# tiantianxuabc/ORB_SLAM2_Refactored

Measured on AMD Instinct MI355X. Metric: frames/sec ORB extract+match (1280×720, 8 lvl, 1000 feat) + LocalBA iters/sec, higher is better.
Workload: dtype u8; 1 GPU; C2: 1280x720 mono, 8 levels, 2000 features, extract + brute-force Hamming top-2/ratio match of every frame vs its predecessor; width=1280, height=720, nlevels=8, nfeatures=2000, parallelism=8192-frame job sharded over 1 GPU(s), 8192 frames per GPU

## Files before the change

### orb_slam2_refactored_amd/csrc/orbx.hip

```cpp
#include <algorithm>
#include <cfloat>
#include <cmath>
#include <cstring>
#include <mutex>
#include <type_traits>
#include <vector>

#include <hip/hip_ext.h>

#include "common.h"
#include "qt_sort.h"
#include "sincos_f.h"
#include "stereo.h"

#include "orbx_geom.h"
#include "orbx_pyramid.h"
#include "orbx_fast.h"
#include "orbx_quadtree.h"
#include "orbx_describe.h"

using namespace orbamd;

struct orbx_extractor {
    orbx_params p;
    int device = 0;
    hipStream_t stream = nullptr;
    std::vector<float> scale, inv_scale, sigma2, inv_sigma2;
    std::vector<int> quota;
    std::mutex mu;

    int g_rows = -1, g_cols = -1;
    Geom geom;
    std::vector<CellDev> cells;
    int NC = 0, PTC = 0;
    size_t qt_lds = 0;
    int qt_ptc0 = 0;
    size_t qt_lds0 = 0;
    int qt_wave = 0, qt_wave_wg = 2, qtw_l0 = 0, qtw_nc = 0, qtw_ptc = 0;
    size_t qtw_lds = 0;
    FastLds fl;
    size_t fast_lds = 0;
    int fast_cpw = 16;
    int fast_spec = 8;
    int fast_pair = 0;
    bool fast_pair_on = false;
    int fast_spec_first = 1;
    int nsub = 1;
    int debug_nc = 0;
    int debug_qt_block = 0;
    uint32_t fault_host = 0;
    int pyr_mfma = 0;
    std::vector<char> pyr_mfma_ok;
    DevBuf d_pyrmt, d_pyrkb;
    int pyr_pair = 2;
    int trig_float = 0;
    int resize_simd = 0;
    std::vector<std::pair<hipStream_t, hipEvent_t>> sub;
    hipEvent_t fork_ev = nullptr;
    bool lvl_overlap = false;
    hipStream_t lvl_side = nullptr;
    hipEvent_t lvl_fork = nullptr, lvl_join = nullptr;
    DevBuf d_cells, d_xtab, d_ytab;
    DevBuf d_strips;
    DevBuf d_slottab;
    DevBuf d_lvlpre;
    std::vector<int> strip_beg;

    int ws_frames = 0;
    DevBuf d_pyr, d_slots, d_cellcnt, d_P, d_T, d_sel, d_selcnt, d_fault;
    DevBuf d_img, d_kps, d_desc, d_counts;
    DevBuf d_stereo_sad;
    void release_buffers() {
        DevBuf* bufs[] = {&d_cells, &d_strips, &d_xtab, &d_ytab, &d_pyr, &d_slots, &d_cellcnt, &d_P,
                          &d_T, &d_sel, &d_selcnt, &d_fault, &d_img, &d_kps, &d_desc,
                          &d_counts, &d_stereo_sad, &d_pyrmt, &d_pyrkb, &d_slottab, &d_lvlpre,
                          &d_stereo_out, &d_dstat};
        for (DevBuf* b : bufs) b->release();
    }
    int prof = 0;
    std::vector<std::pair<hipEvent_t, hipEvent_t>> prof_ev[4];
    std::vector<hipEvent_t> ev_pool;
    const uint8_t* last_in = nullptr;
    long long last_fstride = 0;
    size_t last_step = 0;
    int last_frames = 0;
// ... 44 lines not shown
        nf *= factor;
    }
    h->quota[L - 1] = std::max(p.nfeatures - sum, 0);
}

static int setup_geometry(orbx_extractor* h, int rows, int cols) {
    if (h->g_rows == rows && h->g_cols == cols) return ORB_OK;
    const int Lc = h->p.nlevels;
    Geom g;
    std::memset(&g, 0, sizeof(g));
    g.nlevels = Lc;
    for (int l = Lc; l < MAX_LEVELS; l++) g.lv[l].out_base = INT_MAX;
    std::vector<int2> xtab, ytab;
    std::vector<PyrMfmaLane> mt;
    std::vector<int> mkb;
    std::vector<CellDev> cells;
    long long pyr_off = 0, slot = 0, cand = 0;
    int out = 0, NC = 64;
    int prev_w = cols, prev_h = rows;
    for (int l = 0; l < Lc; l++) {
        LevelDev& L = g.lv[l];
        if (l == 0) {
            L.w = cols; L.h = rows; L.stride = cols; L.off = -1; L.tail_x = cols; L.mt_off = -1;
        } else {
            L.h = cv_round_f(h->inv_scale[l] * rows);
            L.w = cv_round_f(h->inv_scale[l] * cols);
            if (L.w <= 0 || L.h <= 0) {
                set_error("pyramid level collapses to zero size");
                return ORB_EINVAL;
            }
            L.stride = (int)align_up(L.w, 16);
            L.off = pyr_off;
            pyr_off += (long long)align_up((size_t)L.stride * L.h, 256);
            const int sw = prev_w, sh = prev_h, dw = L.w, dh = L.h;
            const double scale_x = 1. / ((double)dw / sw), scale_y = 1. / ((double)dh / sh);
            L.xtab_off = (int)xtab.size();
            L.ytab_off = (int)ytab.size();
            L.ssx = (double)sw / L.w;
            L.ssy = (double)sh / L.h;
            L.tail_x = resize_tail_x(L.w, h->resize_simd);
            int xmax = dw;
            std::vector<int> sxs(dw), a0s(dw), a1s(dw);
            for (int dx = 0; dx < dw; dx++) {
                float fx = (float)((dx + 0.5) * scale_x - 0.5);
                int sx = (int)std::floor(fx);
                fx -= sx;
                if (sx < 0) { fx = 0; sx = 0; }
                if (sx + 1 >= sw) {
                    xmax = std::min(xmax, dx);
                    if (sx >= sw - 1) { fx = 0; sx = sw - 1; }
                }
                sxs[dx] = sx;
                a0s[dx] = std::min(std::max(cv_round_f((1.f - fx) * 2048), -32768), 32767);
                a1s[dx] = std::min(std::max(cv_round_f(fx * 2048), -32768), 32767);
            }
            for (int dx = 0; dx < dw; dx++) {
                int sx0 = sxs[dx], sx1 = std::min(sxs[dx] + 1, sw - 1), a0 = a0s[dx], a1 = a1s[dx];
                if (dx >= xmax) { sx1 = sx0; a0 = 2048; a1 = 0; }
                xtab.push_back(make_int2(sx0 | (sx1 << 16), (a0 & 0xffff) | (a1 << 16)));
            }
            L.mt_off = h->pyr_mfma ? pyr_mfma_tables(xtab.data() + L.xtab_off, dw, mt, mkb) : -1;
            for (int dy = 0; dy < dh; dy++) {
                float fy = (float)((dy + 0.5) * scale_y - 0.5);
                int sy = (int)std::floor(fy);
                fy -= sy;
                const int b0 = std::min(std::max(cv_round_f((1.f - fy) * 2048), -32768), 32767);
                const int b1 = std::min(std::max(cv_round_f(fy * 2048), -32768), 32767);
                auto clip = [&](int y) { return y < 0 ? 0 : (y >= sh ? sh - 1 : y); };
                ytab.push_back(make_int2(clip(sy) | (clip(sy + 1) << 16), (b0 & 0xffff) | (b1 << 16)));
            }
        }
        if (l > 0) {
            const double sc = (double)prev_w / L.w, scy = (double)prev_h / L.h;
            if (sc * PYR_TW + 12 > PYR_SW || scy * PYR_TH + 6 > PYR_SH) {
                set_error("scaleFactor too large for the pyramid tile (max ~1.9)");
                return ORB_EINVAL;
            }
        }
        if (L.w >= 4096 || L.h >= 4096) {
            set_error("image dimensions must be < 4096");
            return ORB_EINVAL;
        }
        prev_w = L.w; prev_h = L.h;
        L.rx = 16; L.ry = 16; L.rw = L.w - 32; L.rh = L.h - 32;
        L.scale = h->scale[l];
        L.size = h->scale[l] * 31;
        L.quota = h->quota[l];
        L.cell_base = (int)cells.size();
        L.ncells = 0;
        L.cand_base = cand;
        L.cand_cap = 0;
        L.nroots = 0;
        L.out_base = out;
        L.out_cap = 0;
        if (L.rw > 0 && L.rh > 0) {
            const int gridw = L.rw / 30, gridh = L.rh / 30;
            if (gridw > 0 && gridh > 0) {
                const int cellw = (int)std::ceil(1. * L.rw / gridw), cellh = (int)std::ceil(1. * L.rh / gridh);
                const int maxx = L.rx + L.rw, maxy = L.ry + L.rh;
                for (int cy = 0, y0 = L.ry; cy < gridh && y0 + 6 < maxy; cy++, y0 += cellh)
                    for (int cx = 0, x0 = L.rx; cx < gridw && x0 + 6 < maxx; cx++, x0 += cellw) {
                        const int y1 = std::min(y0 + cellh + 6, maxy), x1 = std::min(x0 + cellw + 6, maxx);
                        const int zw = x1 - x0 - 6, zh = y1 - y0 - 6;
// ... 90 lines not shown
            h->qtw_nc = ncw;
            h->qtw_ptc = ptcw;
            h->qtw_lds = 4 * ((size_t)ncw * QT_NODE_BYTES + (size_t)ptcw * 8);
            if (h->qtw_lds > 48 * 1024)
                ORB_HIP_TRY(hipFuncSetAttribute((const void*)quadtree_kernel<true>, hipFuncAttributeMaxDynamicSharedMemorySize,
                                                (int)h->qtw_lds));
        }
    }
    int rc;
    if ((rc = h->d_cells.reserve(std::max<size_t>(1, cells.size()) * sizeof(CellDev)))) return rc;
    if ((rc = h->d_xtab.reserve(std::max<size_t>(1, xtab.size()) * sizeof(int2)))) return rc;
    if ((rc = h->d_ytab.reserve(std::max<size_t>(1, ytab.size()) * sizeof(int2)))) return rc;
    if (!cells.empty())
        ORB_HIP_TRY(hipMemcpy(h->d_cells.ptr, cells.data(), cells.size() * sizeof(CellDev), hipMemcpyHostToDevice));
    if (!xtab.empty())
        ORB_HIP_TRY(hipMemcpy(h->d_xtab.ptr, xtab.data(), xtab.size() * sizeof(int2), hipMemcpyHostToDevice));
    if (!ytab.empty())
        ORB_HIP_TRY(hipMemcpy(h->d_ytab.ptr, ytab.data(), ytab.size() * sizeof(int2), hipMemcpyHostToDevice));
    {
        std::vector<uint32_t> st((size_t)g.out_frame, 0u);
        for (int l = 0; l < Lc; l++)
            for (int i = 0; i < g.lv[l].out_cap; i++) st[(size_t)g.lv[l].out_base + i] = (uint32_t)l | ((uint32_t)i << 8);
        if ((rc = h->d_slottab.reserve(st.size() * sizeof(uint32_t)))) return rc;
        ORB_HIP_TRY(hipMemcpy(h->d_slottab.ptr, st.data(), st.size() * sizeof(uint32_t), hipMemcpyHostToDevice));
    }
    if (!mt.empty() && (rc = h->d_pyrmt.reserve(mt.size() * sizeof(PyrMfmaLane)))) return rc;
    if (!mkb.empty() && (rc = h->d_pyrkb.reserve(mkb.size() * sizeof(int)))) return rc;
    if (!mt.empty())
        ORB_HIP_TRY(hipMemcpy(h->d_pyrmt.ptr, mt.data(), mt.size() * sizeof(PyrMfmaLane), hipMemcpyHostToDevice));
    if (!mkb.empty())
        ORB_HIP_TRY(hipMemcpy(h->d_pyrkb.ptr, mkb.data(), mkb.size() * sizeof(int), hipMemcpyHostToDevice));
    h->pyr_mfma_ok.assign(Lc, 0);
    for (int l = 1; l + 1 < Lc; l++) h->pyr_mfma_ok[l] = h->pyr_mfma && pyr_mfma_pair_fits(g, l, mkb, ytab);
    h->geom = g;
    h->cells = cells;
    {
        std::vector<int2> strips;
        h->strip_beg.assign(g.nlevels + 1, 0);
        const int cpw = std::max(1, std::min(h->fast_cpw, 255));
        for (int l = 0; l < g.nlevels; l++) {
            h->strip_beg[l] = (int)strips.size();
            const LevelDev& L = g.lv[l];
            if (L.ncells <= 0) continue;
            const int x00 = cells[L.cell_base].x0y0 & 0xffff;
            int ncx = 0;
            while (ncx < L.ncells && (cells[L.cell_base + ncx].x0y0 >> 16) == (cells[L.cell_base].x0y0 >> 16)) ncx++;
            const int ncy = L.ncells / ncx;
            if (ncx * ncy != L.ncells || (cells[L.cell_base + ncx - 1].x0y0 & 0xffff) < x00) {
                set_error("FAST cell grid is not a rectangle");
                return ORB_EINTERNAL;
            }
            for (int rb = 0; rb < ncy; rb += cpw)
                for (int cx = 0; cx < ncx; cx++) {
                    const int c0 = L.cell_base + rb * ncx + cx, n = std::min(cpw, ncy - rb);
                    for (int k = 1; k < n; k++)
                        if ((cells[c0 + k * ncx].zwzh & 0xffff) != (cells[c0].zwzh & 0xffff)) {
                            set_error("FAST strip with unequal zone widths");
                            return ORB_EINTERNAL;
                        }
                    strips.push_back(make_int2(c0, n | (ncx << 8)));
                }
        }
        h->strip_beg[g.nlevels] = (int)strips.size();
        if ((rc = h->d_strips.reserve(std::max<size_t>(1, strips.size()) * sizeof(int2)))) return rc;
        if (!strips.empty())
            ORB_HIP_TRY(hipMemcpy(h->d_strips.ptr, strips.data(), strips.size() * sizeof(int2), hipMemcpyHostToDevice));
// ... 133 lines not shown
    const unsigned qt_block = h->debug_qt_block ? (unsigned)h->debug_qt_block : (unsigned)QT_THREADS;
    auto quadtree = [&](int l0, int nl, hipStream_t s) {
        if (nl <= 0) return;
        const int lw = std::max(l0, h->qtw_l0), nw_lv = l0 + nl - lw;
        if (nw_lv > 0) {
            launch_timed(h, 2, quadtree_kernel<true>, dim3((unsigned)F, (unsigned)((nw_lv + 3) / 4)), dim3(qt_block),
                         (uint32_t)h->qtw_lds, s, g, cellcnt, slots, h->d_cells.as<CellDev>(), Pb, Tb, sel, selcnt, h->qtw_nc,
                         h->qtw_ptc, fault, lw, nw_lv);
            nl -= nw_lv;
            if (nl <= 0) return;
        }
        if (h->qt_ptc0 > 0 && l0 == 0) {
            launch_timed(h, 2, quadtree_kernel<false>, dim3((unsigned)F, 1u), dim3(qt_block), (uint32_t)h->qt_lds0, s, g,
                         cellcnt, slots, h->d_cells.as<CellDev>(), Pb, Tb, sel, selcnt, h->NC, h->qt_ptc0, fault, 0, 1);
            l0 = 1;
            if (--nl <= 0) return;
        }
        launch_timed(h, 2, quadtree_kernel<false>, dim3((unsigned)F, (unsigned)nl), dim3(qt_block), (uint32_t)h->qt_lds, s,
                     g, cellcnt, slots, h->d_cells.as<CellDev>(), Pb, Tb, sel, selcnt, h->NC, h->PTC, fault, l0, nl);
    };
    auto pyramid = [&](int l) -> int {
        const int first = h->pyr_pair == 2 ? 1 : 2;
        const bool a16 = l > 1 || (((uintptr_t)d_imgs | (uintptr_t)fstride | (uintptr_t)step) & 15) == 0;
        const bool pair = h->pyr_pair && l >= first && (l - first) % 2 == 0 && l + 1 < g.nlevels && a16;
        auto tiles = [&](int lt) {
            return dim3((unsigned)((g.lv[lt].w + PYR_TW - 1) / PYR_TW), (unsigned)((g.lv[lt].h + PYR_TH - 1) / PYR_TH),
                        (unsigned)F);
        };
        if (pair && h->pyr_mfma && h->pyr_mfma_ok[l]) {
            launch_timed(h, 0, pyramid_pair_mfma_kernel, tiles(l + 1), dim3(256), 0u, st, g, l, d_imgs, fstride, step, pyr,
                         h->d_ytab.as<int2>(), h->d_pyrmt.as<PyrMfmaLane>(), h->d_pyrkb.as<int>());
            return 1;
        }
        if (pair && pyr_pair_fits(g, l)) {
            launch_timed(h, 0, pyramid_pair_kernel, tiles(l + 1), dim3(256), 0u, st, g, l, d_imgs, fstride, step, pyr,
                         h->d_xtab.as<int2>(), h->d_ytab.as<int2>());
            return 1;
        }
        launch_timed(h, 0, pyramid_level_kernel, tiles(l), dim3(256), 0u, st, g, l, d_imgs, fstride, step, pyr,
                     h->d_xtab.as<int2>(), h->d_ytab.as<int2>());
        return 0;
    };
    const int nc0 = g.lv[0].ncells;
    if (side && nc0 > 0 && g.nlevels > 1) {
        (void)hipStreamWaitEvent(side, h->lvl_fork, 0);
        fast(0, 1, side);
        quadtree(0, 1, side);
        (void)hipEventRecord(h->lvl_join, side);
        {
            for (int l = 1; l < g.nlevels; l++) l += pyramid(l);
        }
        fast(1, g.nlevels, st);
        quadtree(1, g.nlevels - 1, st);
        (void)hipStreamWaitEvent(st, h->lvl_join, 0);
    } else {
        {
            for (int l = 1; l < g.nlevels; l++) l += pyramid(l);
        }
        fast(0, g.nlevels, st);
        quadtree(0, g.nlevels, st);
    }
    int* lvlpre = h->d_lvlpre.as<int>() + (long long)f0 * LVP;
    hipLaunchKernelGGL(describe_prefix_kernel, dim3((unsigned)((F + 255) / 256)), dim3(256), 0, st, (const int*)selcnt,
                       g.nlevels, F, lvlpre, d_counts, h->d_dstat.as<int>());
    const int rows_max = std::min(g.out_frame, cap);
    const int C = h->desc_dense ? std::max(1, std::min(h->desc_c > 0 ? h->desc_c : rows_max, rows_max)) : 0;
    DescGrid dg{};
    if (C > 0) {
        dg.C = C;
// ... 599 lines not shown
```

### orb_slam2_refactored_amd/csrc/orbx_pyramid.h

```cpp
#pragma once
#include <cmath>
#include <type_traits>
#include <vector>

#include "orbx_geom.h"

namespace orbamd {

typedef unsigned short us2 __attribute__((ext_vector_type(2)));

__device__ __forceinline__ uint32_t htap24(uint32_t h) { return h & 0xffff0u; }
__device__ __forceinline__ uint32_t mulhi24(uint32_t a, uint32_t b) {
    uint32_t r;
    asm("v_mul_hi_u32_u24 %0, %1, %2" : "=v"(r) : "v"(a), "v"(b));
    return r;
}
__device__ __forceinline__ uint32_t vcoef24(int b) { return ((uint32_t)b & 0xfffu) << 12; }
__device__ __forceinline__ uint32_t vtail(uint32_t h0, uint32_t h1, uint32_t b0_24, uint32_t b1_24) {
    return (__umul24(h0, b0_24 >> 12) + __umul24(h1, b1_24 >> 12) + (1u << 21)) >> 22;
}

__device__ __forceinline__ us2 pyr_tap(uint32_t hi, uint32_t lo, uint32_t sel) {
    const uint32_t r = __builtin_amdgcn_perm(hi, lo, sel);
    return *reinterpret_cast<const us2*>(&r);
}

constexpr int PYR_TW = 64, PYR_TH = 64;
constexpr int PYR_SW = 144, PYR_SH = 128;

__device__ __forceinline__ int4 pyr_row_taps(int2 yv, int sy_lo) {
    return make_int4(((yv.x & 0xffff) - sy_lo) * PYR_SW, ((yv.x >> 16) - sy_lo) * PYR_SW, (int)vcoef24(yv.y),
                     (int)vcoef24(yv.y >> 16));
}

__device__ __forceinline__ void pyr_tile_compute(const Geom& g, const LevelDev& L, int f, uint8_t* pyr,
                                                 const uint8_t* S, const int2* xs_t, const int4* ys_t, int tx0,
                                                 int ty0, int tw, int th, int xa) {
    {
        const int q0 = (threadIdx.x & 15) * 4;
        uint32_t sel0[2], sel1[2];
        int wdb[2];
        us2 a0[2], a1[2];
        bool fits = true;
#pragma unroll
        for (int j = 0; j < 2; j++) {
            const int2 xv0 = xs_t[min(q0 + 2 * j, tw - 1)], xv1 = xs_t[min(q0 + 2 * j + 1, tw - 1)];
            const int s00 = (xv0.x & 0xffff) - xa, s01 = (xv0.x >> 16) - xa;
            const int s10 = (xv1.x & 0xffff) - xa, s11 = (xv1.x >> 16) - xa;
            const int wd = s00 >> 2;
            const int e00 = s00 - 4 * wd, e01 = s01 - 4 * wd, e10 = s10 - 4 * wd, e11 = s11 - 4 * wd;
            fits = fits && max(e01, e11) <= 7 && min(e00, e10) >= 0;
            sel0[j] = (uint32_t)e00 | 0x0c00u | ((uint32_t)e01 << 16) | 0x0c000000u;
            sel1[j] = (uint32_t)e10 | 0x0c00u | ((uint32_t)e11 << 16) | 0x0c000000u;
            wdb[j] = 4 * wd;
            a0[j] = *reinterpret_cast<const us2*>(&xv0.y);
            a1[j] = *reinterpret_cast<const us2*>(&xv1.y);
        }
        if (!__syncthreads_or(!fits)) {
            if (q0 >= tw) return;
            const bool full = q0 + 3 < tw;
            uint8_t* dst = pyr + (long long)f * g.pyr_frame_bytes + L.off + tx0 + q0 +
// ... 37 lines not shown
            return;
        }
    }
    const int q0 = (threadIdx.x & 15) * 4;
    if (q0 >= tw) return;
    uint8_t* dbase = pyr + (long long)f * g.pyr_frame_bytes + L.off + tx0 + q0;
#pragma nounroll
    for (int ty = threadIdx.x >> 4; ty < th; ty += 16) {
        const int4 yv = ys_t[ty];
        const int r0 = yv.x, r1 = yv.y;
        const int b0 = yv.z >> 12, b1 = yv.w >> 12;
        uint32_t packed = 0;
#pragma nounroll
        for (int k = 0; k < 4; k++) {
            const int2 xv = xs_t[min(q0 + k, tw - 1)];
            const int sx0 = (xv.x & 0xffff) - xa, sx1 = (xv.x >> 16) - xa, a0 = xv.y & 0xffff, a1 = xv.y >> 16;
            const int h0 = S[r0 + sx0] * a0 + S[r0 + sx1] * a1;
            const int h1 = S[r1 + sx0] * a0 + S[r1 + sx1] * a1;
            const int s0 = min(h0 >> 4, 32767), s1 = min(h1 >> 4, 32767);
            int v = (((s0 * b0) >> 16) + ((s1 * b1) >> 16) + 2) >> 2;
            if (tx0 + q0 + k >= L.tail_x) v = (h0 * b0 + h1 * b1 + (1 << 21)) >> 22;
            packed |= (uint32_t)(v > 255 ? 255 : v) << (8 * k);
        }
        uint8_t* dst = dbase + (long long)(ty0 + ty) * L.stride;
        if (q0 + 3 < tw) *reinterpret_cast<uint32_t*>(dst) = packed;
        else {
            dst[0] = (uint8_t)packed;
            if (q0 + 1 < tw) dst[1] = (uint8_t)(packed >> 8);
            if (q0 + 2 < tw) dst[2] = (uint8_t)(packed >> 16);
        }
    }
}

constexpr int PYR_PF = 5;

struct PyrTile {
    int f, tx0, ty0, tw, th, sy_lo, xa, nc, items, mul;
    const uint8_t* src;
    int sstep;
};

__device__ __forceinline__ PyrTile pyr_tile_geom(const Geom& g, int l, int t, int ntx, int nty, const uint8_t* in,
                                                 long long in_fstride, int in_step, uint8_t* pyr) {
    const LevelDev& L = g.lv[l];
    const LevelDev& Ls = g.lv[l - 1];
    PyrTile T;
    const int per = ntx * nty;
    T.f = t / per;
    const int r = t - T.f * per;
    T.ty0 = (r / ntx) * PYR_TH;
    T.tx0 = (r - (r / ntx) * ntx) * PYR_TW;
    T.tw = min(PYR_TW, L.w - T.tx0);
    T.th = min(PYR_TH, L.h - T.ty0);
    const int sx_lo = max(0, (int)floor((T.tx0 + 0.5) * L.ssx - 0.5) - 2);
    const int sx_hi = min(Ls.w - 1, (int)floor((T.tx0 + T.tw - 0.5) * L.ssx - 0.5) + 2);
    T.sy_lo = max(0, (int)floor((T.ty0 + 0.5) * L.ssy - 0.5) - 2);
    const int sy_hi = min(Ls.h - 1, (int)floor((T.ty0 + T.th - 0.5) * L.ssy - 0.5) + 2);
    T.xa = sx_lo & ~15;
    T.nc = ((sx_hi - T.xa) >> 4) + 1;
    T.items = (sy_hi - T.sy_lo + 1) * T.nc;
    T.mul = ((1 << 20) + T.nc - 1) / T.nc;
    T.src = level_base(g, l - 1, T.f, in, in_fstride, in_step, pyr, &T.sstep);
    auto u = [](int x) { return __builtin_amdgcn_readfirstlane(x); };
    T.f = u(T.f), T.tx0 = u(T.tx0), T.ty0 = u(T.ty0), T.tw = u(T.tw), T.th = u(T.th), T.sy_lo = u(T.sy_lo);
    T.xa = u(T.xa), T.nc = u(T.nc), T.items = u(T.items), T.mul = u(T.mul), T.sstep = u(T.sstep);
    const unsigned long long sp = (unsigned long long)(uintptr_t)T.src;
    T.src = (const uint8_t*)(uintptr_t)(((unsigned long long)(unsigned)u((int)(sp >> 32)) << 32) |
                                        (unsigned)u((int)(unsigned)sp));
    return T;
}

__device__ __forceinline__ int pyr_piece_row(const PyrTile& T, int i) {
    return (int)(__umulhi(((unsigned)i & 0x7ffu) << 12, (unsigned)T.mul & 0xffffffu) & 0x7ffu);
}
__device__ __forceinline__ int mul12(int a, int b) {
    return (int)(((unsigned)a & 0xfffu) * ((unsigned)b & 0xfffu));
}
__device__ __forceinline__ void pyr_piece_load(const PyrTile& T, int i, uint4& v) {
    if (i < T.items) {
        const int rr = pyr_piece_row(T, i), c = i - mul12(rr, T.nc);
        v = *reinterpret_cast<const uint4*>(T.src + __mul24(T.sy_lo + rr, T.sstep) + T.xa + 16 * c);
    }
}

__device__ __forceinline__ void pyr_fetch(const PyrTile& T, int tid, uint4& v0, uint4& v1, uint4& v2, uint4& v3,
                                          uint4& v4) {
    static_assert(PYR_PF == 5, "five pieces per thread");
    pyr_piece_load(T, tid, v0);
    pyr_piece_load(T, tid + 256, v1);
    pyr_piece_load(T, tid + 512, v2);
    pyr_piece_load(T, tid + 768, v3);
    pyr_piece_load(T, tid + 1024, v4);
}

__device__ __forceinline__ void pyr_stage(const PyrTile& T, int tid, uint8_t* S, const uint4& v, int k) {
    const int i = tid + 256 * k;
    if (i < T.items) {
        const int rr = pyr_piece_row(T, i), c = i - mul12(rr, T.nc);
        *reinterpret_cast<uint4*>(&S[mul12(rr, PYR_SW) + 16 * c]) = v;
    }
}

__global__ __launch_bounds__(256) void pyramid_level_kernel(Geom g, int l, const uint8_t* __restrict__ in,
                                                            long long in_fstride, int in_step, uint8_t* pyr,
                                                            const int2* __restrict__ xtab,
                                                            const int2* __restrict__ ytab) {
    __shared__ __attribute__((aligned(16))) uint8_t S[PYR_SH * PYR_SW + 16];
    __shared__ int2 xs_t[PYR_TW];
    __shared__ int4 ys_t[PYR_TH];
    const LevelDev& L = g.lv[l];
    const LevelDev& Ls = g.lv[l - 1];
    const int gx = gridDim.x, gxy = gridDim.x * gridDim.y;
    const int lb = xcd_swizzle(blockIdx.x + gx * blockIdx.y + gxy * blockIdx.z, gxy * gridDim.z);
    const int f = lb / gxy;
    const int tx0 = (lb % gx) * PYR_TW, ty0 = ((lb % gxy) / gx) * PYR_TH;
    const int tw = min(PYR_TW, L.w - tx0), th = min(PYR_TH, L.h - ty0);
    int sstep;
    const uint8_t* src = level_base(g, l - 1, f, in, in_fstride, in_step, pyr, &sstep);
    const int2* xt = xtab + L.xtab_off;
    const int2* yt = ytab + L.ytab_off;
    const int sw = Ls.w, sh = Ls.h;
    const double scx = L.ssx, scy = L.ssy;
    const int sx_lo = max(0, (int)floor((tx0 + 0.5) * scx - 0.5) - 2);
    const int sx_hi = min(sw - 1, (int)floor((tx0 + tw - 0.5) * scx - 0.5) + 2);
    const int sy_lo = max(0, (int)floor((ty0 + 0.5) * scy - 0.5) - 2);
    if ((int)threadIdx.x < tw) xs_t[threadIdx.x] = xt[tx0 + threadIdx.x];
    if ((int)threadIdx.x >= 64 && (int)threadIdx.x - 64 < th)
        ys_t[threadIdx.x - 64] = pyr_row_taps(yt[ty0 + threadIdx.x - 64], sy_lo);
    const int sy_hi = min(sh - 1, (int)floor((ty0 + th - 0.5) * scy - 0.5) + 2);
    const int xa = sx_lo & ~3;
    const int nd = (sx_hi - xa + 4) >> 2;
    const int nr = sy_hi - sy_lo + 1;
    const bool aligned = ((reinterpret_cast<uintptr_t>(src) | (uintptr_t)sstep) & 3) == 0;
    if (((reinterpret_cast<uintptr_t>(src) | (uintptr_t)sstep) & 15) == 0 && sx_hi - (sx_lo & ~15) < PYR_SW) {
        const PyrTile T = pyr_tile_geom(g, l, lb, gx, gridDim.y, in, in_fstride, in_step, pyr);
        uint4 v0, v1, v2, v3, v4;
        pyr_fetch(T, threadIdx.x, v0, v1, v2, v3, v4);
        pyr_stage(T, threadIdx.x, S, v0, 0);
        pyr_stage(T, threadIdx.x, S, v1, 1);
        pyr_stage(T, threadIdx.x, S, v2, 2);
        pyr_stage(T, threadIdx.x, S, v3, 3);
        pyr_stage(T, threadIdx.x, S, v4, 4);
        __syncthreads();
        pyr_tile_compute(g, L, f, pyr, S, xs_t, ys_t, tx0, ty0, tw, th, T.xa);
        return;
    }
    if (aligned) {
        constexpr int RPW = PYR_SH / 4;
        const int wv = __builtin_amdgcn_readfirstlane((int)(threadIdx.x >> 6));
        const int ln = threadIdx.x & 63;
        const int col = min(xa + 4 * ln, (sw - 1) & ~3);
        const uint8_t* rbase = src + (long long)sy_lo * sstep + col;
        uint32_t v[RPW];
#pragma unroll
        for (int k = 0; k < RPW; k++) {
            const int rk = min(wv + 4 * k, nr - 1);
            v[k] = *reinterpret_cast<const uint32_t*>(rbase + (long long)rk * sstep);
        }
        if (ln < nd) {
            uint32_t* drow = reinterpret_cast<uint32_t*>(S) + wv * (PYR_SW / 4) + ln;
#pragma unroll
            for (int k = 0; k < RPW; k++)
                if (wv + 4 * k < nr) drow[k * PYR_SW] = v[k];
        }
    } else {
        for (int i = threadIdx.x; i < nd * nr; i += blockDim.x) {
            const int r = i / nd, d = i - r * nd;
            const uint8_t* rowp = src + (long long)(sy_lo + r) * sstep;
            const int x = xa + 4 * d;
            uint32_t v = 0;
            for (int q = 0; q < 4; q++)
                if (x + q < sw) v |= (uint32_t)rowp[x + q] << (8 * q);
            *reinterpret_cast<uint32_t*>(&S[r * PYR_SW + 4 * d]) = v;
        }
    }
    __syncthreads();
    pyr_tile_compute(g, L, f, pyr, S, xs_t, ys_t, tx0, ty0, tw, th, xa);
}

constexpr int PP_MAXP = 8;
constexpr int PP_MAXC = 96, PP_MAXR = 96;

__device__ __forceinline__ uint32_t pyr_px_generic(const uint8_t* S, int2 xv, int4 yv, int xa, bool tail) {
    const int r0 = yv.x, r1 = yv.y;
    const int sx0 = (xv.x & 0xffff) - xa, sx1 = (xv.x >> 16) - xa, a0 = xv.y & 0xffff, a1 = xv.y >> 16;
    const int b0 = yv.z >> 12, b1 = yv.w >> 12;
    const int h0 = S[r0 + sx0] * a0 + S[r0 + sx1] * a1;
    const int h1 = S[r1 + sx0] * a0 + S[r1 + sx1] * a1;
    const int s0 = min(h0 >> 4, 32767), s1 = min(h1 >> 4, 32767);
    int v = (((s0 * b0) >> 16) + ((s1 * b1) >> 16) + 2) >> 2;
    if (tail) v = (h0 * b0 + h1 * b1 + (1 << 21)) >> 22;
    return (uint32_t)(v > 255 ? 255 : v);
}

__global__ __launch_bounds__(256) void pyramid_pair_kernel(Geom g, int l, const uint8_t* __restrict__ in,
                                                           long long in_fstride, int in_step, uint8_t* pyr,
                                                           const int2* __restrict__ xtab,
                                                           const int2* __restrict__ ytab) {
    __shared__ __attribute__((aligned(16))) uint8_t S[PYR_SH * PYR_SW + 16];
    __shared__ int2 xs1[PP_MAXC], xs2[PYR_TW];
    __shared__ int4 ys1[PP_MAXR], ys2[PYR_TH];
    const LevelDev& L0 = g.lv[l - 1];
    const LevelDev& L1 = g.lv[l];
    const LevelDev& L2 = g.lv[l + 1];
    const int tid = threadIdx.x;
    const int gx = gridDim.x, gxy = gridDim.x * gridDim.y;
    const int lb = xcd_swizzle(blockIdx.x + gx * blockIdx.y + gxy * blockIdx.z, gxy * gridDim.z);
    const int f = lb / gxy;
    const int tx0 = (lb % gx) * PYR_TW, ty0 = ((lb % gxy) / gx) * PYR_TH;
    const int tw = min(PYR_TW, L2.w - tx0), th = min(PYR_TH, L2.h - ty0);
    auto u = [](int x) { return __builtin_amdgcn_readfirstlane(x); };
    const int ax0 = max(0, (int)floor((tx0 + 0.5) * L2.ssx - 0.5) - 2);
    const int c1 = u(min(L1.w - 1, (int)floor((tx0 + tw - 0.5) * L2.ssx - 0.5) + 2));
    const int ay0 = u(max(0, (int)floor((ty0 + 0.5) * L2.ssy - 0.5) - 2));
    const int ay1 = u(min(L1.h - 1, (int)floor((ty0 + th - 0.5) * L2.ssy - 0.5) + 2));
    const int c0 = u(ax0 & ~3);
    const int ncol = c1 - c0 + 1, nrow = ay1 - ay0 + 1;
    PyrTile T;
    const int bx0 = max(0, (int)floor((c0 + 0.5) * L1.ssx - 0.5) - 2);
    const int bx1 = min(L0.w - 1, (int)floor((c1 + 0.5) * L1.ssx - 0.5) + 2);
    T.sy_lo = u(max(0, (int)floor((ay0 + 0.5) * L1.ssy - 0.5) - 2));
    const int by1 = min(L0.h - 1, (int)floor((ay1 + 0.5) * L1.ssy - 0.5) + 2);
    T.xa = u(bx0 & ~15);
    T.nc = u(((bx1 - T.xa) >> 4) + 1);
    T.items = u((by1 - T.sy_lo + 1) * T.nc);
    T.mul = u(((1 << 20) + T.nc - 1) / T.nc);
    T.src = level_base(g, l - 1, f, in, in_fstride, in_step, pyr, &T.sstep);
    {
        uint4 v0, v1, v2, v3, v4;
        pyr_fetch(T, tid, v0, v1, v2, v3, v4);
        if (tid < ncol) xs1[tid] = xtab[L1.xtab_off + c0 + tid];
        if (tid < nrow) ys1[tid] = pyr_row_taps(ytab[L1.ytab_off + ay0 + tid], T.sy_lo);
        if (tid < tw) xs2[tid] = xtab[L2.xtab_off + tx0 + tid];
        if (tid < th) ys2[tid] = pyr_row_taps(ytab[L2.ytab_off + ty0 + tid], ay0);
        pyr_stage(T, tid, S, v0, 0);
        pyr_stage(T, tid, S, v1, 1);
        pyr_stage(T, tid, S, v2, 2);
        pyr_stage(T, tid, S, v3, 3);
        pyr_stage(T, tid, S, v4, 4);
    }
    __syncthreads();
    const int ncq = (ncol + 3) >> 2, rpp = 256 / ncq;
    const int q = tid % ncq, r0 = tid / ncq;
    const bool act = r0 < rpp;
    uint32_t out[PP_MAXP];
    if (act) {
        uint32_t sel0[2], sel1[2], wdv[2];
        us2 a0[2], a1[2];
        int2 xv[4];
        bool fits = true;
#pragma unroll
        for (int k = 0; k < 4; k++) xv[k] = xs1[min(4 * q + k, ncol - 1)];
#pragma unroll
        for (int j = 0; j < 2; j++) {
            const int2 xv0 = xv[2 * j], xv1 = xv[2 * j + 1];
            const int s00 = (xv0.x & 0xffff) - T.xa, s01 = (xv0.x >> 16) - T.xa;
            const int s10 = (xv1.x & 0xffff) - T.xa, s11 = (xv1.x >> 16) - T.xa;
            const int wd = s00 >> 2;
            const int e00 = s00 - 4 * wd, e01 = s01 - 4 * wd, e10 = s10 - 4 * wd, e11 = s11 - 4 * wd;
            fits = fits && max(e01, e11) <= 7 && min(e00, e10) >= 0;
            sel0[j] = (uint32_t)e00 | 0x0c00u | ((uint32_t)e01 << 16) | 0x0c000000u;
            sel1[j] = (uint32_t)e10 | 0x0c00u | ((uint32_t)e11 << 16) | 0x0c000000u;
            wdv[j] = (uint32_t)wd;
            a0[j] = *reinterpret_cast<const us2*>(&xv0.y);
            a1[j] = *reinterpret_cast<const us2*>(&xv1.y);
        }
        const int tcol = L1.tail_x - (c0 + 4 * q);
        auto rows = [&](auto tail_c) {
            constexpr bool TAIL = decltype(tail_c)::value;
#pragma unroll
            for (int pp = 0; pp < PP_MAXP; pp++) {
                const int r = r0 + pp * rpp;
                out[pp] = 0;
                if (r >= nrow) break;
                const int4 yv = ys1[r];
                if (fits) {
                    const uint32_t b0 = (uint32_t)yv.z, b1 = (uint32_t)yv.w;
#pragma unroll
                    for (int j = 0; j < 2; j++) {
                        const uint32_t* s0 = reinterpret_cast<const uint32_t*>(S + yv.x + 4 * (int)wdv[j]);
                        const uint32_t* s1 = reinterpret_cast<const uint32_t*>(S + yv.y + 4 * (int)wdv[j]);
                        const uint32_t w00 = s0[0], w01 = s0[1], w10 = s1[0], w11 = s1[1];
                        const uint32_t r0a = __builtin_amdgcn_udot2(pyr_tap(w01, w00, sel0[j]), a0[j], 0u, false);
                        const uint32_t r1a = __builtin_amdgcn_udot2(pyr_tap(w11, w10, sel0[j]), a0[j], 0u, false);
                        const uint32_t r0b = __builtin_amdgcn_udot2(pyr_tap(w01, w00, sel1[j]), a1[j], 0u, false);
                        const uint32_t r1b = __builtin_amdgcn_udot2(pyr_tap(w11, w10, sel1[j]), a1[j], 0u, false);
                        uint32_t va = (mulhi24(htap24(r0a), b0) + mulhi24(htap24(r1a), b1) + 2) >> 2;
                        uint32_t vb = (mulhi24(htap24(r0b), b0) + mulhi24(htap24(r1b), b1) + 2) >> 2;
                        if (TAIL) {
                            va = 2 * j >= tcol ? vtail(r0a, r1a, b0, b1) : va;
                            vb = 2 * j + 1 >= tcol ? vtail(r0b, r1b, b0, b1) : vb;
                        }
                        out[pp] |= (va | (vb << 8)) << (16 * j);
                    }
                } else {
#pragma unroll
                    for (int k = 0; k < 4; k++) out[pp] |= pyr_px_generic(S, xv[k], yv, T.xa, k >= tcol) << (8 * k);
                }
            }
        };
        if (c1 >= L1.tail_x) rows(std::true_type{});
        else
            rows(std::false_type{});
    }
    __syncthreads();
    if (act) {
        uint8_t* lrow = pyr + (long long)f * g.pyr_frame_bytes + L1.off + c0 + 4 * q;
        const bool full = c0 + 4 * q + 3 <= c1;
#pragma unroll
        for (int pp = 0; pp < PP_MAXP; pp++) {
            const int r = r0 + pp * rpp;
            if (r >= nrow) break;
            *reinterpret_cast<uint32_t*>(&S[r * PYR_SW + 4 * q]) = out[pp];
            uint8_t* dst = lrow + __mul24(ay0 + r, L1.stride);
            if (full) {
                *reinterpret_cast<uint32_t*>(dst) = out[pp];
            } else {
                for (int k = 0; k < 3; k++)
                    if (c0 + 4 * q + k <= c1) dst[k] = (uint8_t)(out[pp] >> (8 * k));
            }
        }
    }
    __syncthreads();
    pyr_tile_compute(g, L2, f, pyr, S, xs2, ys2, tx0, ty0, tw, th, c0);
}

static bool pyr_pair_fits(const Geom& g, int l) {
    const double s1x = g.lv[l].ssx, s1y = g.lv[l].ssy, s2x = g.lv[l + 1].ssx, s2y = g.lv[l + 1].ssy;
    const int ncol = (int)std::ceil(PYR_TW * s2x) + 10, nrow = (int)std::ceil(PYR_TH * s2y) + 7;
    const int ncq = (ncol + 3) / 4, rpp = 256 / ncq;
    const int bw = (int)std::ceil(ncol * s1x) + 7 + 15, bh = (int)std::ceil(nrow * s1y) + 7;
    return ncol + 8 <= PYR_SW && nrow <= PYR_SH && ncol <= PP_MAXC && nrow <= PP_MAXR && (nrow + rpp - 1) / rpp <= PP_MAXP &&
           bw <= PYR_SW && bh <= PYR_SH &&
           bh * ((bw + 15) / 16) <= PYR_PF * 256;
}

typedef _Float16 h8v __attribute__((ext_vector_type(8)));
typedef float pf4v __attribute__((ext_vector_type(4)));
struct PyrMfmaLane { uint32_t a[4]; float c[4]; };
constexpr int PM_MAXB1 = 6;
constexpr int PM_TAB = PYR_SH;
constexpr int PM_MAXU1 = 12;


template <bool TAIL>
__device__ __forceinline__ uint32_t pyr_mfma_unit(const uint8_t* sp, int k, const h8v& A, const pf4v& C, const int4& t,
                                                  int tcol) {
    const int g = lane_id() >> 4;
    constexpr uint32_t hmask = TAIL ? 0xfffffu : 0xffff0u;
    const uint2 w = *reinterpret_cast<const uint2*>(sp + k * (15 * PYR_SW));
    const uint4 bu = make_uint4(__builtin_amdgcn_perm(0x64646464u, w.x, 0x04010400u),
                                __builtin_amdgcn_perm(0x64646464u, w.x, 0x04030402u),
                                __builtin_amdgcn_perm(0x64646464u, w.y, 0x04010400u),
                                __builtin_amdgcn_perm(0x64646464u, w.y, 0x04030402u));
    const pf4v d = __builtin_amdgcn_mfma_f32_16x16x32_f16(A, __builtin_bit_cast(h8v, bu), C, 0, 0, 0);
    const uint32_t b0 = (uint32_t)t.y, b1 = (uint32_t)t.z;
    uint32_t out = 0;
#pragma unroll
    for (int j = 0; j < 4; j++) {
        const uint32_t h0 = __float_as_uint(d[j]) & hmask;
        const uint32_t h1 = (uint32_t)__builtin_amdgcn_mov_dpp((int)h0, 0x101, 0xf, 0xf, true);
        uint32_t v;
        if (!TAIL) {
            v = (mulhi24(h0, b0) + mulhi24(h1, b1) + 2) >> 2;
        } else {
            v = (mulhi24(h0 & 0xffff0u, b0) + mulhi24(h1 & 0xffff0u, b1) + 2) >> 2;
            v = 4 * g + j >= tcol ? vtail(h0, h1, b0, b1) : v;
// ... 256 lines not shown
```

Measured before the change: 174,400 frames/s.

## Derive pyramid tile source rects from resize tables and template pair kernel passes

Pyramid tile source spans are now read from the precomputed x/y resize tap tables instead of being recomputed with double-precision floor math on the device. Pair-kernel eligibility is checked on the host by walking every tile's exact rectangle, and that check also yields the pass count. The pair kernel is templated on the pass count so a 7-pass variant needs fewer output registers. Integer divisions are replaced by a constant-memory reciprocal table. The aim is less per-tile address arithmetic and lower register pressure, at the cost of more host-side planning code and possible tile-rect differences if the tables and the old formula disagree.

```diff
diff --git a/orb_slam2_refactored_amd/csrc/orbx.hip b/orb_slam2_refactored_amd/csrc/orbx.hip
--- a/orb_slam2_refactored_amd/csrc/orbx.hip
+++ b/orb_slam2_refactored_amd/csrc/orbx.hip
@@ -51,6 +51,7 @@
     uint32_t fault_host = 0;
     int pyr_mfma = 0;
     std::vector<char> pyr_mfma_ok;
+    std::vector<int> pyr_pair_np;
     DevBuf d_pyrmt, d_pyrkb;
     int pyr_pair = 2;
     int trig_float = 0;
@@ -161,43 +162,13 @@
             L.stride = (int)align_up(L.w, 16);
             L.off = pyr_off;
             pyr_off += (long long)align_up((size_t)L.stride * L.h, 256);
-            const int sw = prev_w, sh = prev_h, dw = L.w, dh = L.h;
-            const double scale_x = 1. / ((double)dw / sw), scale_y = 1. / ((double)dh / sh);
             L.xtab_off = (int)xtab.size();
             L.ytab_off = (int)ytab.size();
-            L.ssx = (double)sw / L.w;
-            L.ssy = (double)sh / L.h;
+            L.ssx = (double)prev_w / L.w;
+            L.ssy = (double)prev_h / L.h;
             L.tail_x = resize_tail_x(L.w, h->resize_simd);
-            int xmax = dw;
-            std::vector<int> sxs(dw), a0s(dw), a1s(dw);
-            for (int dx = 0; dx < dw; dx++) {
-                float fx = (float)((dx + 0.5) * scale_x - 0.5);
-                int sx = (int)std::floor(fx);
-                fx -= sx;
-                if (sx < 0) { fx = 0; sx = 0; }
-                if (sx + 1 >= sw) {
-                    xmax = std::min(xmax, dx);
-                    if (sx >= sw - 1) { fx = 0; sx = sw - 1; }
-                }
-                sxs[dx] = sx;
-                a0s[dx] = std::min(std::max(cv_round_f((1.f - fx) * 2048), -32768), 32767);
-                a1s[dx] = std::min(std::max(cv_round_f(fx * 2048), -32768), 32767);
-            }
-            for (int dx = 0; dx < dw; dx++) {
-                int sx0 = sxs[dx], sx1 = std::min(sxs[dx] + 1, sw - 1), a0 = a0s[dx], a1 = a1s[dx];
-                if (dx >= xmax) { sx1 = sx0; a0 = 2048; a1 = 0; }
-                xtab.push_back(make_int2(sx0 | (sx1 << 16), (a0 & 0xffff) | (a1 << 16)));
-            }
-            L.mt_off = h->pyr_mfma ? pyr_mfma_tables(xtab.data() + L.xtab_off, dw, mt, mkb) : -1;
-            for (int dy = 0; dy < dh; dy++) {
-                float fy = (float)((dy + 0.5) * scale_y - 0.5);
-                int sy = (int)std::floor(fy);
-                fy -= sy;
-                const int b0 = std::min(std::max(cv_round_f((1.f - fy) * 2048), -32768), 32767);
-                const int b1 = std::min(std::max(cv_round_f(fy * 2048), -32768), 32767);
-                auto clip = [&](int y) { return y < 0 ? 0 : (y >= sh ? sh - 1 : y); };
-                ytab.push_back(make_int2(clip(sy) | (clip(sy + 1) << 16), (b0 & 0xffff) | (b1 << 16)));
-            }
+            pyr_resize_tables(prev_w, prev_h, L.w, L.h, xtab, ytab);
+            L.mt_off = h->pyr_mfma ? pyr_mfma_tables(xtab.data() + L.xtab_off, L.w, mt, mkb) : -1;
         }
         if (l > 0) {
             const double sc = (double)prev_w / L.w, scy = (double)prev_h / L.h;
@@ -354,6 +325,8 @@
         ORB_HIP_TRY(hipMemcpy(h->d_pyrkb.ptr, mkb.data(), mkb.size() * sizeof(int), hipMemcpyHostToDevice));
     h->pyr_mfma_ok.assign(Lc, 0);
     for (int l = 1; l + 1 < Lc; l++) h->pyr_mfma_ok[l] = h->pyr_mfma && pyr_mfma_pair_fits(g, l, mkb, ytab);
+    h->pyr_pair_np.assign(Lc, 0);
+    for (int l = 1; l + 1 < Lc; l++) h->pyr_pair_np[l] = pyr_pair_fits(g, l, xtab, ytab);
     h->geom = g;
     h->cells = cells;
     {
@@ -553,9 +526,9 @@
                          h->d_ytab.as<int2>(), h->d_pyrmt.as<PyrMfmaLane>(), h->d_pyrkb.as<int>());
             return 1;
         }
-        if (pair && pyr_pair_fits(g, l)) {
-            launch_timed(h, 0, pyramid_pair_kernel, tiles(l + 1), dim3(256), 0u, st, g, l, d_imgs, fstride, step, pyr,
-                         h->d_xtab.as<int2>(), h->d_ytab.as<int2>());
+        if (pair && h->pyr_pair_np[l]) {
+            launch_timed(h, 0, h->pyr_pair_np[l] <= 7 ? pyramid_pair_kernel<7> : pyramid_pair_kernel<PP_MAXP>, tiles(l + 1),
+                         dim3(256), 0u, st, g, l, d_imgs, fstride, step, pyr, h->d_xtab.as<int2>(), h->d_ytab.as<int2>());
             return 1;
         }
         launch_timed(h, 0, pyramid_level_kernel, tiles(l), dim3(256), 0u, st, g, l, d_imgs, fstride, step, pyr,
diff --git a/orb_slam2_refactored_amd/csrc/orbx_pyr_rect.h b/orb_slam2_refactored_amd/csrc/orbx_pyr_rect.h
--- /dev/null
+++ b/orb_slam2_refactored_amd/csrc/orbx_pyr_rect.h
@@ -0,0 +1,137 @@
+#pragma once
+#include <algorithm>
+#include <cmath>
+#include <vector>
+
+#if defined(__HIPCC__)
+#define PYR_HD __host__ __device__ __forceinline__
+#else
+#define PYR_HD inline
+#endif
+
+namespace orbamd {
+
+constexpr int PYR_TW = 64, PYR_TH = 64;
+constexpr int PYR_SW = 144, PYR_SH = 128;
+constexpr int PYR_PF = 5;
+constexpr int PP_MAXP = 8;
+constexpr int PP_MAXC = 96, PP_MAXR = 96;
+constexpr int PYR_RECIP_N = PP_MAXC / 4 + 1;
+
+template <class T2>
+inline void pyr_resize_tables(int sw, int sh, int dw, int dh, std::vector<T2>& xtab, std::vector<T2>& ytab) {
+    auto coef = [](float v) { return std::min(std::max((int)std::lrintf(v), -32768), 32767); };
+    auto entry = [](int a, int b) {
+        T2 v;
+        v.x = a, v.y = b;
+        return v;
+    };
+    const double scale_x = 1. / ((double)dw / sw), scale_y = 1. / ((double)dh / sh);
+    int xmax = dw;
+    std::vector<int> sxs(dw), a0s(dw), a1s(dw);
+    for (int dx = 0; dx < dw; dx++) {
+        float fx = (float)((dx + 0.5) * scale_x - 0.5);
+        int sx = (int)std::floor(fx);
+        fx -= sx;
+        if (sx < 0) { fx = 0; sx = 0; }
+        if (sx + 1 >= sw) {
+            xmax = std::min(xmax, dx);
+            if (sx >= sw - 1) { fx = 0; sx = sw - 1; }
+        }
+        sxs[dx] = sx;
+        a0s[dx] = coef((1.f - fx) * 2048);
+        a1s[dx] = coef(fx * 2048);
+    }
+    for (int dx = 0; dx < dw; dx++) {
+        int sx0 = sxs[dx], sx1 = std::min(sxs[dx] + 1, sw - 1), a0 = a0s[dx], a1 = a1s[dx];
+        if (dx >= xmax) { sx1 = sx0; a0 = 2048; a1 = 0; }
+        xtab.push_back(entry(sx0 | (sx1 << 16), (a0 & 0xffff) | (a1 << 16)));
+    }
+    for (int dy = 0; dy < dh; dy++) {
+        float fy = (float)((dy + 0.5) * scale_y - 0.5);
+        int sy = (int)std::floor(fy);
+        fy -= sy;
+        const int b0 = coef((1.f - fy) * 2048), b1 = coef(fy * 2048);
+        auto clip = [&](int y) { return y < 0 ? 0 : (y >= sh ? sh - 1 : y); };
+        ytab.push_back(entry(clip(sy) | (clip(sy + 1) << 16), (b0 & 0xffff) | (b1 << 16)));
+    }
+}
+
+struct PyrSpan { int lo, hi; };
+template <class T2>
+PYR_HD PyrSpan pyr_tap_span(const T2* tab, int i0, int i1) {
+    return PyrSpan{(int)(tab[i0].x & 0xffff), (int)((unsigned)tab[i1].x >> 16)};
+}
+
+struct PyrPairRect { int c0, c1, ay0, ay1, xa, bx1, by0, by1; };
+template <class T2>
+PYR_HD PyrPairRect pyr_pair_rect(const T2* xt1, const T2* yt1, const T2* xt2, const T2* yt2, int tx0, int ty0,
+                                 int tw, int th) {
+    const PyrSpan ax = pyr_tap_span(xt2, tx0, tx0 + tw - 1), ay = pyr_tap_span(yt2, ty0, ty0 + th - 1);
+    PyrPairRect R;
+    R.c0 = ax.lo & ~3, R.c1 = ax.hi, R.ay0 = ay.lo, R.ay1 = ay.hi;
+    const PyrSpan bx = pyr_tap_span(xt1, R.c0, R.c1), by = pyr_tap_span(yt1, R.ay0, R.ay1);
+    R.xa = bx.lo & ~15, R.bx1 = bx.hi, R.by0 = by.lo, R.by1 = by.hi;
+    return R;
+}
+
+constexpr unsigned pyr_recip20(int n) { return (unsigned)(((1 << 20) + n - 1) / n); }
+
+struct PyrCaps { int tw, th, sw, sh, maxc, maxr, maxp, pieces; };
+constexpr PyrCaps PYR_CAPS{PYR_TW, PYR_TH, PYR_SW, PYR_SH, PP_MAXC, PP_MAXR, PP_MAXP, PYR_PF * 256};
+struct PyrPairPlan {
+    bool ok;
+    int passes, max_ncol, max_nrow;
+    long long slots, pixels;
+};
+template <class T2>
+inline PyrPairPlan pyr_pair_plan(int w0, int h0, int w1, int h1, int w2, int h2, const T2* xt1, const T2* yt1,
+                                 const T2* xt2, const T2* yt2, const PyrCaps& K = PYR_CAPS) {
+    PyrPairPlan P{false, 0, 0, 0, 0, (long long)w1 * h1 + (long long)w2 * h2};
+    auto lo = [](const T2& v) { return (int)(v.x & 0xffff); };
+    auto hi = [](const T2& v) { return (int)((unsigned)v.x >> 16); };
+    auto inside = [&](const T2* tab, int i0, int i1, PyrSpan s, int n) {
+        if (s.lo < 0 || s.hi >= n || s.lo > s.hi) return false;
+        for (int i = i0; i <= i1; i++)
+            if (lo(tab[i]) < s.lo || hi(tab[i]) > s.hi || lo(tab[i]) > hi(tab[i])) return false;
+        return true;
+    };
+    const int tw_max = K.tw, th_max = K.th;
+    if (tw_max % 4 || tw_max < 4 || tw_max > 256 || th_max < 1) return P;
+    const int rpp2 = 256 / (tw_max / 4);
+    int covx = 0, covy = 0;
+    for (int ty0 = 0; ty0 < h2; ty0 += th_max) {
+        const int th = std::min(th_max, h2 - ty0);
+        int covx_row = 0;
+        for (int tx0 = 0; tx0 < w2; tx0 += tw_max) {
+            const int tw = std::min(tw_max, w2 - tx0);
+            const PyrPairRect R = pyr_pair_rect(xt1, yt1, xt2, yt2, tx0, ty0, tw, th);
+            if (!inside(xt2, tx0, tx0 + tw - 1, PyrSpan{R.c0, R.c1}, w1) ||
+                !inside(yt2, ty0, ty0 + th - 1, PyrSpan{R.ay0, R.ay1}, h1) ||
+                !inside(xt1, R.c0, R.c1, PyrSpan{R.xa, R.bx1}, w0) || !inside(yt1, R.ay0, R.ay1, PyrSpan{R.by0, R.by1}, h0))
+                return P;
+            const int ncol = R.c1 - R.c0 + 1, nrow = R.ay1 - R.ay0 + 1;
+            const int ncq = (ncol + 3) / 4, rpp = 256 / ncq, np = (nrow + rpp - 1) / rpp;
+            const int nc = ((R.bx1 - R.xa) >> 4) + 1, bh = R.by1 - R.by0 + 1;
+            if (4 * ncq + 8 > K.sw || nrow > K.sh || ncol > K.maxc || nrow > K.maxr || np > K.maxp || 16 * nc > K.sw ||
+                bh > K.sh || bh * nc > K.pieces)
+                return P;
+            if (R.c0 > covx_row || R.ay0 > covy) return P;
+            covx_row = std::max(covx_row, R.c1 + 1);
+            if (tx0 + tw == w2) {
+                if (covx_row != w1) return P;
+                covx = w1;
+            }
+            if (tx0 + tw == w2 && ty0 + th == h2 && R.ay1 + 1 != h1) return P;
+            P.passes = std::max(P.passes, np);
+            P.max_ncol = std::max(P.max_ncol, ncol);
+            P.max_nrow = std::max(P.max_nrow, nrow);
+            P.slots += 1024ll * np + 1024ll * ((th + rpp2 - 1) / rpp2);
+            if (tx0 + tw == w2) covy = std::max(covy, R.ay1 + 1);
+        }
+    }
+    P.ok = covx == w1 && covy == h1 && P.passes >= 1;
+    return P;
+}
+
+}
diff --git a/orb_slam2_refactored_amd/csrc/orbx_pyramid.h b/orb_slam2_refactored_amd/csrc/orbx_pyramid.h
--- a/orb_slam2_refactored_amd/csrc/orbx_pyramid.h
+++ b/orb_slam2_refactored_amd/csrc/orbx_pyramid.h
@@ -4,6 +4,7 @@
 #include <vector>
 
 #include "orbx_geom.h"
+#include "orbx_pyr_rect.h"
 
 namespace orbamd {
 
@@ -25,8 +26,14 @@
     return *reinterpret_cast<const us2*>(&r);
 }
 
-constexpr int PYR_TW = 64, PYR_TH = 64;
-constexpr int PYR_SW = 144, PYR_SH = 128;
+struct PyrRecipTab { unsigned m[PYR_RECIP_N]; };
+constexpr PyrRecipTab pyr_recip_tab() {
+    PyrRecipTab t{};
+    for (int n = 1; n < PYR_RECIP_N; n++) t.m[n] = pyr_recip20(n);
+    return t;
+}
+__constant__ PyrRecipTab c_pyr_recip = pyr_recip_tab();
+static_assert(PYR_SW / 16 < PYR_RECIP_N, "the staging piece counts are in the table");
 
 __device__ __forceinline__ int4 pyr_row_taps(int2 yv, int sy_lo) {
     return make_int4(((yv.x & 0xffff) - sy_lo) * PYR_SW, ((yv.x >> 16) - sy_lo) * PYR_SW, (int)vcoef24(yv.y),
@@ -130,7 +137,6 @@
     }
 }
 
-constexpr int PYR_PF = 5;
 
 struct PyrTile {
     int f, tx0, ty0, tw, th, sy_lo, xa, nc, items, mul;
@@ -138,10 +144,9 @@
     int sstep;
 };
 
-__device__ __forceinline__ PyrTile pyr_tile_geom(const Geom& g, int l, int t, int ntx, int nty, const uint8_t* in,
-                                                 long long in_fstride, int in_step, uint8_t* pyr) {
+__device__ __forceinline__ PyrTile pyr_tile_geom(const Geom& g, int l, int t, int ntx, int nty, PyrSpan sx, PyrSpan sy,
+                                                 const uint8_t* in, long long in_fstride, int in_step, uint8_t* pyr) {
     const LevelDev& L = g.lv[l];
-    const LevelDev& Ls = g.lv[l - 1];
     PyrTile T;
     const int per = ntx * nty;
     T.f = t / per;
@@ -150,14 +155,11 @@
     T.tx0 = (r - (r / ntx) * ntx) * PYR_TW;
     T.tw = min(PYR_TW, L.w - T.tx0);
     T.th = min(PYR_TH, L.h - T.ty0);
-    const int sx_lo = max(0, (int)floor((T.tx0 + 0.5) * L.ssx - 0.5) - 2);
-    const int sx_hi = min(Ls.w - 1, (int)floor((T.tx0 + T.tw - 0.5) * L.ssx - 0.5) + 2);
-    T.sy_lo = max(0, (int)floor((T.ty0 + 0.5) * L.ssy - 0.5) - 2);
-    const int sy_hi = min(Ls.h - 1, (int)floor((T.ty0 + T.th - 0.5) * L.ssy - 0.5) + 2);
-    T.xa = sx_lo & ~15;
-    T.nc = ((sx_hi - T.xa) >> 4) + 1;
-    T.items = (sy_hi - T.sy_lo + 1) * T.nc;
-    T.mul = ((1 << 20) + T.nc - 1) / T.nc;
+    T.sy_lo = sy.lo;
+    T.xa = sx.lo & ~15;
+    T.nc = ((sx.hi - T.xa) >> 4) + 1;
+    T.items = (sy.hi - sy.lo + 1) * T.nc;
+    T.mul = (int)c_pyr_recip.m[T.nc];
     T.src = level_base(g, l - 1, T.f, in, in_fstride, in_step, pyr, &T.sstep);
     auto u = [](int x) { return __builtin_amdgcn_readfirstlane(x); };
     T.f = u(T.f), T.tx0 = u(T.tx0), T.ty0 = u(T.ty0), T.tw = u(T.tw), T.th = u(T.th), T.sy_lo = u(T.sy_lo);
@@ -217,21 +219,20 @@
     const uint8_t* src = level_base(g, l - 1, f, in, in_fstride, in_step, pyr, &sstep);
     const int2* xt = xtab + L.xtab_off;
     const int2* yt = ytab + L.ytab_off;
-    const int sw = Ls.w, sh = Ls.h;
-    const double scx = L.ssx, scy = L.ssy;
-    const int sx_lo = max(0, (int)floor((tx0 + 0.5) * scx - 0.5) - 2);
-    const int sx_hi = min(sw - 1, (int)floor((tx0 + tw - 0.5) * scx - 0.5) + 2);
-    const int sy_lo = max(0, (int)floor((ty0 + 0.5) * scy - 0.5) - 2);
+    const int sw = Ls.w;
+    const PyrSpan sx = pyr_tap_span(xt, tx0, tx0 + tw - 1), sy = pyr_tap_span(yt, ty0, ty0 + th - 1);
+    const int sx_lo = __builtin_amdgcn_readfirstlane(sx.lo), sx_hi = __builtin_amdgcn_readfirstlane(sx.hi);
+    const int sy_lo = __builtin_amdgcn_readfirstlane(sy.lo), sy_hi = __builtin_amdgcn_readfirstlane(sy.hi);
     if ((int)threadIdx.x < tw) xs_t[threadIdx.x] = xt[tx0 + threadIdx.x];
     if ((int)threadIdx.x >= 64 && (int)threadIdx.x - 64 < th)
         ys_t[threadIdx.x - 64] = pyr_row_taps(yt[ty0 + threadIdx.x - 64], sy_lo);
-    const int sy_hi = min(sh - 1, (int)floor((ty0 + th - 0.5) * scy - 0.5) + 2);
     const int xa = sx_lo & ~3;
     const int nd = (sx_hi - xa + 4) >> 2;
     const int nr = sy_hi - sy_lo + 1;
     const bool aligned = ((reinterpret_cast<uintptr_t>(src) | (uintptr_t)sstep) & 3) == 0;
     if (((reinterpret_cast<uintptr_t>(src) | (uintptr_t)sstep) & 15) == 0 && sx_hi - (sx_lo & ~15) < PYR_SW) {
-        const PyrTile T = pyr_tile_geom(g, l, lb, gx, gridDim.y, in, in_fstride, in_step, pyr);
+        const PyrTile T = pyr_tile_geom(g, l, lb, gx, gridDim.y, PyrSpan{sx_lo, sx_hi}, PyrSpan{sy_lo, sy_hi}, in,
+                                        in_fstride, in_step, pyr);
         uint4 v0, v1, v2, v3, v4;
         pyr_fetch(T, threadIdx.x, v0, v1, v2, v3, v4);
         pyr_stage(T, threadIdx.x, S, v0, 0);
@@ -276,8 +277,6 @@
     pyr_tile_compute(g, L, f, pyr, S, xs_t, ys_t, tx0, ty0, tw, th, xa);
 }
 
-constexpr int PP_MAXP = 8;
-constexpr int PP_MAXC = 96, PP_MAXR = 96;
 
 __device__ __forceinline__ uint32_t pyr_px_generic(const uint8_t* S, int2 xv, int4 yv, int xa, bool tail) {
     const int r0 = yv.x, r1 = yv.y;
@@ -291,6 +290,7 @@
     return (uint32_t)(v > 255 ? 255 : v);
 }
 
+template <int NP>
 __global__ __launch_bounds__(256) void pyramid_pair_kernel(Geom g, int l, const uint8_t* __restrict__ in,
                                                            long long in_fstride, int in_step, uint8_t* pyr,
                                                            const int2* __restrict__ xtab,
@@ -298,7 +298,6 @@
     __shared__ __attribute__((aligned(16))) uint8_t S[PYR_SH * PYR_SW + 16];
     __shared__ int2 xs1[PP_MAXC], xs2[PYR_TW];
     __shared__ int4 ys1[PP_MAXR], ys2[PYR_TH];
-    const LevelDev& L0 = g.lv[l - 1];
     const LevelDev& L1 = g.lv[l];
     const LevelDev& L2 = g.lv[l + 1];
     const int tid = threadIdx.x;
@@ -308,21 +307,16 @@
     const int tx0 = (lb % gx) * PYR_TW, ty0 = ((lb % gxy) / gx) * PYR_TH;
     const int tw = min(PYR_TW, L2.w - tx0), th = min(PYR_TH, L2.h - ty0);
     auto u = [](int x) { return __builtin_amdgcn_readfirstlane(x); };
-    const int ax0 = max(0, (int)floor((tx0 + 0.5) * L2.ssx - 0.5) - 2);
-    const int c1 = u(min(L1.w - 1, (int)floor((tx0 + tw - 0.5) * L2.ssx - 0.5) + 2));
-    const int ay0 = u(max(0, (int)floor((ty0 + 0.5) * L2.ssy - 0.5) - 2));
-    const int ay1 = u(min(L1.h - 1, (int)floor((ty0 + th - 0.5) * L2.ssy - 0.5) + 2));
-    const int c0 = u(ax0 & ~3);
+    const PyrPairRect R = pyr_pair_rect(xtab + L1.xtab_off, ytab + L1.ytab_off, xtab + L2.xtab_off,
+                                        ytab + L2.ytab_off, tx0, ty0, tw, th);
+    const int c0 = u(R.c0), c1 = u(R.c1), ay0 = u(R.ay0), ay1 = u(R.ay1);
     const int ncol = c1 - c0 + 1, nrow = ay1 - ay0 + 1;
     PyrTile T;
-    const int bx0 = max(0, (int)floor((c0 + 0.5) * L1.ssx - 0.5) - 2);
-    const int bx1 = min(L0.w - 1, (int)floor((c1 + 0.5) * L1.ssx - 0.5) + 2);
-    T.sy_lo = u(max(0, (int)floor((ay0 + 0.5) * L1.ssy - 0.5) - 2));
-    const int by1 = min(L0.h - 1, (int)floor((ay1 + 0.5) * L1.ssy - 0.5) + 2);
-    T.xa = u(bx0 & ~15);
-    T.nc = u(((bx1 - T.xa) >> 4) + 1);
-    T.items = u((by1 - T.sy_lo + 1) * T.nc);
-    T.mul = u(((1 << 20) + T.nc - 1) / T.nc);
+    T.sy_lo = u(R.by0);
+    T.xa = u(R.xa);
+    T.nc = u(((R.bx1 - R.xa) >> 4) + 1);
+    T.items = u((R.by1 - R.by0 + 1) * T.nc);
+    T.mul = u((int)c_pyr_recip.m[T.nc]);
     T.src = level_base(g, l - 1, f, in, in_fstride, in_step, pyr, &T.sstep);
     {
         uint4 v0, v1, v2, v3, v4;
@@ -338,10 +332,12 @@
         pyr_stage(T, tid, S, v4, 4);
     }
     __syncthreads();
-    const int ncq = (ncol + 3) >> 2, rpp = 256 / ncq;
-    const int q = tid % ncq, r0 = tid / ncq;
+    const int ncq = (ncol + 3) >> 2;
+    const unsigned m20 = (unsigned)u((int)c_pyr_recip.m[ncq]);
+    const int rpp = (int)(m20 >> 12);
+    const int r0 = (int)(__umul24((unsigned)tid, m20) >> 20), q = tid - __mul24(r0, ncq);
     const bool act = r0 < rpp;
-    uint32_t out[PP_MAXP];
+    uint32_t out[NP];
     if (act) {
         uint32_t sel0[2], sel1[2], wdv[2];
         us2 a0[2], a1[2];
@@ -367,10 +363,11 @@
         auto rows = [&](auto tail_c) {
             constexpr bool TAIL = decltype(tail_c)::value;
 #pragma unroll
-            for (int pp = 0; pp < PP_MAXP; pp++) {
+            for (int pp = 0; pp < NP; pp++) {
                 const int r = r0 + pp * rpp;
                 out[pp] = 0;
-                if (r >= nrow) break;
+                if (pp * rpp >= nrow) break;
+                if ((pp + 1) * rpp > nrow && r >= nrow) break;
                 const int4 yv = ys1[r];
                 if (fits) {
                     const uint32_t b0 = (uint32_t)yv.z, b1 = (uint32_t)yv.w;
@@ -406,9 +403,10 @@
         uint8_t* lrow = pyr + (long long)f * g.pyr_frame_bytes + L1.off + c0 + 4 * q;
         const bool full = c0 + 4 * q + 3 <= c1;
 #pragma unroll
-        for (int pp = 0; pp < PP_MAXP; pp++) {
+        for (int pp = 0; pp < NP; pp++) {
             const int r = r0 + pp * rpp;
-            if (r >= nrow) break;
+            if (pp * rpp >= nrow) break;
+            if ((pp + 1) * rpp > nrow && r >= nrow) break;
             *reinterpret_cast<uint32_t*>(&S[r * PYR_SW + 4 * q]) = out[pp];
             uint8_t* dst = lrow + __mul24(ay0 + r, L1.stride);
             if (full) {
@@ -423,14 +421,12 @@
     pyr_tile_compute(g, L2, f, pyr, S, xs2, ys2, tx0, ty0, tw, th, c0);
 }
 
-static bool pyr_pair_fits(const Geom& g, int l) {
-    const double s1x = g.lv[l].ssx, s1y = g.lv[l].ssy, s2x = g.lv[l + 1].ssx, s2y = g.lv[l + 1].ssy;
-    const int ncol = (int)std::ceil(PYR_TW * s2x) + 10, nrow = (int)std::ceil(PYR_TH * s2y) + 7;
-    const int ncq = (ncol + 3) / 4, rpp = 256 / ncq;
-    const int bw = (int)std::ceil(ncol * s1x) + 7 + 15, bh = (int)std::ceil(nrow * s1y) + 7;
-    return ncol + 8 <= PYR_SW && nrow <= PYR_SH && ncol <= PP_MAXC && nrow <= PP_MAXR && (nrow + rpp - 1) / rpp <= PP_MAXP &&
-           bw <= PYR_SW && bh <= PYR_SH &&
-           bh * ((bw + 15) / 16) <= PYR_PF * 256;
+static int pyr_pair_fits(const Geom& g, int l, const std::vector<int2>& xtab, const std::vector<int2>& ytab) {
+    const LevelDev &L0 = g.lv[l - 1], &L1 = g.lv[l], &L2 = g.lv[l + 1];
+    const PyrPairPlan P = pyr_pair_plan(L0.w, L0.h, L1.w, L1.h, L2.w, L2.h, xtab.data() + L1.xtab_off,
+                                        ytab.data() + L1.ytab_off, xtab.data() + L2.xtab_off, ytab.data() + L2.ytab_off);
+    if (!P.ok) return 0;
+    return P.passes <= 7 ? 7 : PP_MAXP;
 }
 
 typedef _Float16 h8v __attribute__((ext_vector_type(8)));
```

Result: faster. 177,300 frames/s, median of 6 (+1.7%).
